# ZiyuanMa/MAPF_RL

Hardware: NVIDIA B200
Metric: env_agent_steps_per_sec_step_observe (higher is better)
Workload: dtype u8

## Files before the change

mapf_rl_b200/csrc/mapf_bfs_device.cuh:

```cuda
#pragma once
#include <type_traits>

#include "mapf_common.cuh"

namespace {

#ifdef MAPF_ENABLE_DIAG
__device__ unsigned long long g_bfs_cycles[8];
#endif

template <int RW, int RPL>
struct BfsState {
    uint32_t unv[RPL][RW];
    uint32_t fro[RPL][RW];
    uint32_t m1[RPL][RW];
    uint32_t m2[RPL][RW];
};

__device__ __forceinline__ uint32_t bfs_column_mask(int L, int w)
{
    const int lo = max(4 - 32 * w, 0), hi = min(L + 4 - 32 * w, 32);
    if (hi <= lo) return 0u;
    return (hi - lo == 32) ? 0xffffffffu : (((1u << (hi - lo)) - 1u) << lo);
}

template <int RW, int RPL>
struct BfsFree {
    uint32_t v[RPL][RW];
};

template <int RW, int RPL, int APW>
__device__ __forceinline__ void bfs_load_free(const EnvDims &d, const uint32_t *ob, BfsFree<RW, RPL> &F)
{
    constexpr int LW = 32 / APW;
    const int lane = (threadIdx.x & 31) % LW;
#pragma unroll
    for (int q = 0; q < RPL; ++q) {
        const int row = lane * RPL + q;
#pragma unroll
        for (int w = 0; w < RW; ++w)
            F.v[q][w] = (row < d.L) ? (~__ldcg(ob + (row + 4) * d.RWS + w) & bfs_column_mask(d.L, w)) : 0u;
    }
}

template <int RW, int RPL, int APW>
__device__ __forceinline__ void bfs_init(const EnvDims &d, const BfsFree<RW, RPL> &F, const int gx, const int gy, const bool alive,
                                         BfsState<RW, RPL> &S)
{
    constexpr int LW = 32 / APW;
    const int lane = (threadIdx.x & 31) % LW;
#pragma unroll
    for (int q = 0; q < RPL; ++q) {
        const int row = lane * RPL + q;
#pragma unroll
        for (int w = 0; w < RW; ++w) {
            const uint32_t fre = alive ? F.v[q][w] : 0u;
            const int p = gy + 4;
            S.fro[q][w] = (row == gx && (p >> 5) == w) ? ((1u << (p & 31)) & fre) : 0u;
            S.unv[q][w] = fre & ~S.fro[q][w];
            S.m1[q][w] = S.m2[q][w] = 0;
        }
    }
}

template <int RW, int RPL, int APW, bool WRAP>
__device__ __forceinline__ uint32_t bfs_wave(const BfsState<RW, RPL> &S, uint32_t (&nw)[RPL][RW])
{
    constexpr int LW = 32 / APW;
    const int lane = (threadIdx.x & 31) % LW;
    uint32_t any = 0;
#pragma unroll
    for (int w = 0; w < RW; ++w) {
        uint32_t above, below;
        if constexpr (WRAP) {
            above = __shfl_sync(MAPF_FULL_MASK, S.fro[RPL - 1][w], (lane + LW - 1) & (LW - 1), LW);
            below = __shfl_sync(MAPF_FULL_MASK, S.fro[0][w], (lane + 1) & (LW - 1), LW);
        } else {
            above = __shfl_up_sync(MAPF_FULL_MASK, S.fro[RPL - 1][w], 1, LW);
            below = __shfl_down_sync(MAPF_FULL_MASK, S.fro[0][w], 1, LW);
            if (lane == 0) above = 0;
            if (lane == LW - 1) below = 0;
        }
#pragma unroll
        for (int q = 0; q < RPL; ++q) {
            const uint32_t f = S.fro[q][w];
            const uint32_t fl = w > 0 ? __funnelshift_l(S.fro[q][w > 0 ? w - 1 : 0], f, 1) : f << 1;
            const uint32_t fr = w < RW - 1 ? __funnelshift_r(f, S.fro[q][w < RW - 1 ? w + 1 : w], 1) : f >> 1;
            const uint32_t up = q > 0 ? S.fro[q > 0 ? q - 1 : 0][w] : above;
            const uint32_t dn = q < RPL - 1 ? S.fro[q < RPL - 1 ? q + 1 : q][w] : below;
            const uint32_t x = (fl | fr | up | dn) & S.unv[q][w];
            nw[q][w] = x;
            any |= x;
        }
    }
    return any;
}

template <int RW, int RPL, int SEL>
__device__ __forceinline__ void bfs_apply(BfsState<RW, RPL> &S, const uint32_t (&nw)[RPL][RW])
{
#pragma unroll
    for (int q = 0; q < RPL; ++q)
#pragma unroll
        for (int w = 0; w < RW; ++w) {
            S.unv[q][w] -= nw[q][w];
            S.fro[q][w] = nw[q][w];
            if constexpr (SEL == 1) S.m1[q][w] += nw[q][w];
            if constexpr (SEL == 2) S.m2[q][w] += nw[q][w];
        }
}

template <int RW, int RPL, int APW, bool KEEP>
__device__ __forceinline__ void bfs_emit(const EnvDims &d, const uint32_t *ob, const BfsFree<RW, RPL> &F, const int e, const int a,
                                         const bool alive, const BfsState<RW, RPL> &S, uint32_t *__restrict__ navi)
{
    constexpr int LW = 32 / APW;
    const int lane = (threadIdx.x & 31) % LW;
    uint32_t pl[4][RPL][RW];
    uint32_t z[RPL][RW];
#pragma unroll
    for (int q = 0; q < RPL; ++q) {
        const int row = alive ? lane * RPL + q : d.L;
#pragma unroll
        for (int w = 0; w < RW; ++w) {
            uint32_t fre;
            if constexpr (KEEP) fre = alive ? F.v[q][w] : 0u;
            else fre = (row < d.L) ? (~__ldcg(ob + (row + 4) * d.RWS + w) & bfs_column_mask(d.L, w)) : 0u;
            z[q][w] = fre & ~S.unv[q][w] & ~S.m1[q][w] & ~S.m2[q][w];
        }
    }
    auto closer = [](uint32_t c1, uint32_t c2, uint32_t cz, uint32_t n1, uint32_t n2, uint32_t nz) -> uint32_t {
        return (c1 & nz) | (c2 & n1) | (cz & n2);
    };
#pragma unroll
    for (int w = 0; w < RW; ++w) {
        uint32_t a1 = __shfl_up_sync(MAPF_FULL_MASK, S.m1[RPL - 1][w], 1, LW), b1 = __shfl_down_sync(MAPF_FULL_MASK, S.m1[0][w], 1, LW);
        uint32_t a2 = __shfl_up_sync(MAPF_FULL_MASK, S.m2[RPL - 1][w], 1, LW), b2 = __shfl_down_sync(MAPF_FULL_MASK, S.m2[0][w], 1, LW);
        uint32_t az = __shfl_up_sync(MAPF_FULL_MASK, z[RPL - 1][w], 1, LW), bz = __shfl_down_sync(MAPF_FULL_MASK, z[0][w], 1, LW);
        if (lane == 0) a1 = a2 = az = 0;
        if (lane == LW - 1) b1 = b2 = bz = 0;
#pragma unroll
        for (int q = 0; q < RPL; ++q) {
            auto left = [&](const uint32_t(&m)[RPL][RW]) {
                return w > 0 ? __funnelshift_l(m[q][w > 0 ? w - 1 : 0], m[q][w], 1) : m[q][w] << 1;
            };
            auto right = [&](const uint32_t(&m)[RPL][RW]) {
                return w < RW - 1 ? __funnelshift_r(m[q][w], m[q][w < RW - 1 ? w + 1 : w], 1) : m[q][w] >> 1;
            };
            const uint32_t c1 = S.m1[q][w], c2 = S.m2[q][w], cz = z[q][w];
            const uint32_t u1 = q > 0 ? S.m1[q > 0 ? q - 1 : 0][w] : a1, u2 = q > 0 ? S.m2[q > 0 ? q - 1 : 0][w] : a2,
                           uz = q > 0 ? z[q > 0 ? q - 1 : 0][w] : az;
            const uint32_t d1 = q < RPL - 1 ? S.m1[q < RPL - 1 ? q + 1 : q][w] : b1, d2 = q < RPL - 1 ? S.m2[q < RPL - 1 ? q + 1 : q][w] : b2,
                           dz = q < RPL - 1 ? z[q < RPL - 1 ? q + 1 : q][w] : bz;
            pl[0][q][w] = closer(c1, c2, cz, u1, u2, uz);
            pl[1][q][w] = closer(c1, c2, cz, d1, d2, dz);
            pl[2][q][w] = closer(c1, c2, cz, left(S.m1), left(S.m2), left(z));
            pl[3][q][w] = closer(c1, c2, cz, right(S.m1), right(S.m2), right(z));
        }
    }
    uint2 *nv = reinterpret_cast<uint2 *>(navi + ((size_t)e * d.N + a) * d.navi_agent_stride);
#pragma unroll
    for (int q = 0; q < RPL; ++q) {
        const int row = lane * RPL + q;
        if (row >= d.L || !alive) continue;
        const int pr = row + 4, bx1 = pr >> 3, r1 = pr & 7;
#pragma unroll
        for (int by = 0; by < 4 * RW; ++by) {
            if (by >= d.NB) continue;
            constexpr int kLast = RW - 1;
            const int w = by >> 2;
            const int s = (by & 3) * 8;
            uint32_t f[4];
#pragma unroll
            for (int k = 0; k < 4; ++k)
                f[k] = __funnelshift_r(pl[k][q][w], w < kLast ? pl[k][q][w < kLast ? w + 1 : kLast] : 0u, s) & 0xffffu;
            const uint2 v = make_uint2(f[0] | (f[1] << 16), f[2] | (f[3] << 16));
            if (bx1 < d.NB) nv[((size_t)(bx1 * d.NB + by) << 4) + r1] = v;
            if (bx1 > 0) nv[((size_t)((bx1 - 1) * d.NB + by) << 4) + r1 + 8] = v;
        }
    }
}

template <int RW, int RPL, int APW, bool WRAP, bool DIST, bool KEEP>
__device__ __forceinline__ void bfs_navi_search(const EnvDims &d, const int e, const int a, const int i, const bool alive,
                                                const uint32_t *__restrict__ ob, const BfsFree<RW, RPL> &F, const int gx, const int gy,
                                                uint32_t *__restrict__ navi, int32_t *__restrict__ dist_out)
{
    constexpr int LW = 32 / APW;
    const int lane = (threadIdx.x & 31) % LW;
#ifdef MAPF_ENABLE_DIAG
    const long long tb0 = clock64();
    long long triples = 0;
#endif
    BfsState<RW, RPL> S;
    bfs_init<RW, RPL, APW>(d, F, gx, gy, alive, S);
#ifdef MAPF_ENABLE_DIAG
    const long long tb1 = clock64();
#endif

    int32_t *dist = nullptr;
    if constexpr (DIST) {
        dist = alive ? dist_out + ((size_t)i * d.N + a) * d.L * d.L : nullptr;
        for (int q = 0; q < RPL; ++q) {
            const int row = lane * RPL + q;
            if (dist && row < d.L)
                for (int y = 0; y < d.L; ++y) dist[row * d.L + y] = MAPF_DIST_UNREACHABLE;
        }
        __syncwarp();
#pragma unroll
        for (int q = 0; q < RPL; ++q)
#pragma unroll
            for (int w = 0; w < RW; ++w)
                if (dist && S.fro[q][w]) dist[gx * d.L + gy] = 0;
    }

    auto wave = [&](auto selc, const int t) -> uint32_t {
        constexpr int sel = decltype(selc)::value;
        uint32_t nw[RPL][RW];
        const uint32_t any = bfs_wave<RW, RPL, APW, WRAP>(S, nw);
        bfs_apply<RW, RPL, sel>(S, nw);
        if constexpr (DIST) {
#pragma unroll
            for (int q = 0; q < RPL; ++q)
#pragma unroll
                for (int w = 0; w < RW; ++w) {
                    uint32_t x = dist ? nw[q][w] : 0u;
                    while (x) {
                        int b = __ffs(x) - 1;
                        x &= x - 1;
                        dist[(lane * RPL + q) * d.L + (32 * w + b - 4)] = t;
                    }
                }
        }
        return any;
    };
    for (int t = 1;; t += 3) {
        wave(std::integral_constant<int, 1>{}, t);
        wave(std::integral_constant<int, 2>{}, t + 1);
        const uint32_t any = wave(std::integral_constant<int, 0>{}, t + 2);
#ifdef MAPF_ENABLE_DIAG
        ++triples;
#endif
        if (!__any_sync(MAPF_FULL_MASK, any != 0)) break;
    }
#ifdef MAPF_ENABLE_DIAG
    const long long tb2 = clock64();
#endif
    bfs_emit<RW, RPL, APW, KEEP>(d, ob, F, e, a, alive, S, navi);
#ifdef MAPF_ENABLE_DIAG
    if (e == 0 && (threadIdx.x & 31) == 0) {
        const long long tb3 = clock64();
        atomicAdd(&g_bfs_cycles[0], (unsigned long long)(tb1 - tb0));
        atomicAdd(&g_bfs_cycles[1], (unsigned long long)(tb2 - tb1));
        atomicAdd(&g_bfs_cycles[2], (unsigned long long)(tb3 - tb2));
        atomicAdd(&g_bfs_cycles[3], 1ull);
        atomicAdd(&g_bfs_cycles[4], (unsigned long long)triples);
    }
#endif
}

template <int RW, int RPL, int APW>
__device__ __forceinline__ void bfs_navi_warp(const EnvDims &d, const int e, const int a, const int i, const bool alive,
                                              const uint32_t *__restrict__ obst, const uint8_t *__restrict__ goal,
                                              uint32_t *__restrict__ navi, int32_t *__restrict__ dist_out)
{
    constexpr int LW = 32 / APW;
    const uint32_t *ob = obst + (size_t)e * d.obst_stride;
    const uchar2 gg = __ldcg(reinterpret_cast<const uchar2 *>(goal) + (size_t)e * d.N + a);
    BfsFree<RW, RPL> F;
    bfs_load_free<RW, RPL, APW>(d, ob, F);
    if (dist_out) bfs_navi_search<RW, RPL, APW, false, true, false>(d, e, a, i, alive, ob, F, gg.x, gg.y, navi, dist_out);
    else if (d.L < LW * RPL) bfs_navi_search<RW, RPL, APW, true, false, false>(d, e, a, i, alive, ob, F, gg.x, gg.y, navi, nullptr);
    else bfs_navi_search<RW, RPL, APW, false, false, false>(d, e, a, i, alive, ob, F, gg.x, gg.y, navi, nullptr);
}

template <int RW, int RPL, int APW>
__device__ __forceinline__ void bfs_navi_warp_pre(const EnvDims &d, const int e, const int a, const bool alive, const uint32_t *__restrict__ ob,
                                                  const BfsFree<RW, RPL> &F, const int gx, const int gy, uint32_t *__restrict__ navi)
{
    constexpr int LW = 32 / APW;
    if (d.L < LW * RPL) bfs_navi_search<RW, RPL, APW, true, false, true>(d, e, a, 0, alive, ob, F, gx, gy, navi, nullptr);
    else bfs_navi_search<RW, RPL, APW, false, false, true>(d, e, a, 0, alive, ob, F, gx, gy, navi, nullptr);
}

}
```

mapf_rl_b200/csrc/mapf_reset_device.cuh:

```cuda
#pragma once
#include "mapf_common.cuh"

namespace {


__device__ __forceinline__ uint4 philox4x32_10(uint4 c, uint2 k)
{
#pragma unroll
    for (int r = 0; r < 10; ++r) {
        const uint32_t hi0 = __umulhi(0xD2511F53u, c.x), lo0 = 0xD2511F53u * c.x;
        const uint32_t hi1 = __umulhi(0xCD9E8D57u, c.z), lo1 = 0xCD9E8D57u * c.z;
        c = make_uint4(hi1 ^ c.y ^ k.x, lo1, hi0 ^ c.w ^ k.y, lo0);
        k.x += 0x9E3779B9u;
        k.y += 0xBB67AE85u;
    }
    return c;
}

enum : uint32_t { PURPOSE_DENSITY = 0, PURPOSE_MAP = 1, PURPOSE_AGENT = 2, PURPOSE_LEVEL = 3 };

#ifdef MAPF_ENABLE_DIAG
__device__ unsigned long long g_reset_cycles[8];
#define MAPF_RESET_TICK(slot)                 \
    do {                                      \
        const long long _now = clock64();     \
        _acc[slot] += _now - _t0;             \
        _t0 = _now;                           \
    } while (0)
#else
#define MAPF_RESET_TICK(slot) do {} while (0)
#endif

template <int RW, int RPL>
struct Bits {
    uint32_t v[RPL][RW];
};

template <int RW, int RPL>
__device__ __forceinline__ void dilate(const Bits<RW, RPL> &f, Bits<RW, RPL> &out, int lane)
{
#pragma unroll
    for (int q = 0; q < RPL; ++q)
#pragma unroll
        for (int w = 0; w < RW; ++w) {
            const uint32_t x = f.v[q][w];
            uint32_t fl = x << 1, fr = x >> 1;
            if (w > 0) fl |= f.v[q][w > 0 ? w - 1 : 0] >> 31;
            if (w < RW - 1) fr |= f.v[q][w < RW - 1 ? w + 1 : w] << 31;
            uint32_t up = __shfl_up_sync(MAPF_FULL_MASK, x, 1);
            uint32_t dn = __shfl_down_sync(MAPF_FULL_MASK, x, 1);
            uint32_t wrap_up = 0, wrap_dn = 0;
            if (q > 0) wrap_up = __shfl_sync(MAPF_FULL_MASK, f.v[q > 0 ? q - 1 : 0][w], 31);
            if (q < RPL - 1) wrap_dn = __shfl_sync(MAPF_FULL_MASK, f.v[q < RPL - 1 ? q + 1 : q][w], 0);
            if (lane == 0) up = wrap_up;
            if (lane == 31) dn = wrap_dn;
            out.v[q][w] = fl | fr | up | dn;
        }
}

template <int RW, int RPL>
__device__ __forceinline__ int count_bits(const Bits<RW, RPL> &m)
{
    int c = 0;
#pragma unroll
    for (int q = 0; q < RPL; ++q)
#pragma unroll
        for (int w = 0; w < RW; ++w) c += __popc(m.v[q][w]);
    return c;
}

__device__ __forceinline__ int nth_set_bit(uint32_t m, int n)
{
    int pos = 0;
#pragma unroll
    for (int half = 16; half >= 1; half >>= 1) {
        const int c = __popc(m & ((1u << half) - 1u));
        if (n >= c) {
            n -= c;
            pos += half;
            m >>= half;
        }
    }
    return pos;
}

template <int RW, int RPL>
__device__ __forceinline__ int pick_bit(const Bits<RW, RPL> &m, uint32_t rnd, int lane, int &total_out)
{
    constexpr int kMax = 32 * RW * RPL;
    constexpr int kBits = kMax >= 512 ? 10 : (kMax >= 256 ? 9 : (kMax >= 128 ? 8 : (kMax >= 64 ? 7 : 6)));
    const int c = count_bits(m);
    const uint32_t lt = (1u << lane) - 1u;
    int excl = 0, total = 0;
#pragma unroll
    for (int k = 0; k < kBits; ++k) {
        const uint32_t b = __ballot_sync(MAPF_FULL_MASK, (c >> k) & 1);
        excl += __popc(b & lt) << k;
        total += __popc(b) << k;
    }
    total_out = total;
    if (total == 0) return -1;
    const int r = (int)__umulhi(rnd, (uint32_t)total);
    int local = r - excl;
    uint32_t code = 0;
    if (local >= 0 && local < c) {
        bool found = false;
#pragma unroll
        for (int q = 0; q < RPL; ++q)
#pragma unroll
            for (int w = 0; w < RW; ++w) {
                const int pc = __popc(m.v[q][w]);
                if (!found && local < pc) {
                    code = (uint32_t)((((lane + 32 * q) << 8) | (32 * w + nth_set_bit(m.v[q][w], local))) + 1);
                    found = true;
                }
                if (!found) local -= pc;
            }
    }
    return (int)__reduce_or_sync(MAPF_FULL_MASK, code) - 1;
}

template <int RW, int RPL>
__device__ __forceinline__ void clear_cell(Bits<RW, RPL> &m, int code, int lane)
{
    const int row = code >> 8, col = code & 0xff;
#pragma unroll
    for (int q = 0; q < RPL; ++q)
#pragma unroll
        for (int w = 0; w < RW; ++w)
            if (lane + 32 * q == row && (col >> 5) == w) m.v[q][w] &= ~(1u << (col & 31));
}

template <int RW, int RPL>
__device__ __forceinline__ bool test_cell(const Bits<RW, RPL> &m, int code, int lane)
{
    const int row = code >> 8, col = code & 0xff;
    bool hit = false;
#pragma unroll
    for (int q = 0; q < RPL; ++q)
#pragma unroll
        for (int w = 0; w < RW; ++w)
            if (lane + 32 * q == row && (col >> 5) == w) hit = (m.v[q][w] >> (col & 31)) & 1u;
    return __any_sync(MAPF_FULL_MASK, hit);
}

template <int RW, int RPL>
__device__ __forceinline__ void reset_env_warp(const EnvDims &d, const int e, const uint64_t seed, const uint64_t g,
                                               const float density, uint32_t *__restrict__ obst, uint8_t *__restrict__ pos,
                                               uint8_t *__restrict__ goal, int32_t *__restrict__ steps, int32_t *__restrict__ err,
                                               const int L, const int N)
{
    const int lane = threadIdx.x & 31;
    const int NS = d.N;
    const uint2 key = make_uint2((uint32_t)seed, (uint32_t)(seed >> 32));
    const uint32_t g_lo = (uint32_t)g, g_hi = (uint32_t)(g >> 32);

    float dens = density;
    if (density < 0.f) {
        const uint4 r = philox4x32_10(make_uint4(g_lo, g_hi, PURPOSE_DENSITY, 0u), key);
        const float u = (float)(r.x >> 8) * (1.0f / 16777216.0f);
        dens = u < 0.66f ? sqrtf(u * 0.5f * 0.33f) : 0.5f - sqrtf((1.0f - u) * 0.5f * 0.17f);
    }
    const uint32_t thresh = dens <= 0.f ? 0u : (dens >= 1.f ? 0xffffffffu : (uint32_t)((double)dens * 4294967296.0));

    Bits<RW, RPL> fre, elig, comp, big;
    int big_n = 0;
#ifdef MAPF_ENABLE_DIAG
    long long _t0 = clock64();
    long long _acc[8] = {0, 0, 0, 0, 0, 0, 0, 0};
#endif
    for (uint32_t attempt = 0;; ++attempt) {
        if (attempt >= 256) {
            if (lane == 0) atomicOr(err, MAPF_ERRBIT_RESET);
            break;
        }
#pragma unroll
        for (int q = 0; q < RPL; ++q) {
            const int row = lane + 32 * q;
#pragma unroll
            for (int w = 0; w < RW; ++w) fre.v[q][w] = 0;
            if (row < L) {
                for (int y4 = 0; y4 < L; y4 += 4) {
                    const uint4 r = philox4x32_10(make_uint4(g_lo, g_hi, PURPOSE_MAP | (attempt << 8), (uint32_t)(row * 64 + (y4 >> 2))), key);
                    uint32_t nib = (r.x >= thresh ? 1u : 0u) | (r.y >= thresh ? 2u : 0u) | (r.z >= thresh ? 4u : 0u) | (r.w >= thresh ? 8u : 0u);
                    if (y4 + 4 > L) nib &= (1u << (L - y4)) - 1u;
                    const int p = y4 + 4;
#pragma unroll
                    for (int w = 0; w < RW; ++w)
                        if ((p >> 5) == w) fre.v[q][w] |= nib << (p & 31);
                }
            }
        }
        MAPF_RESET_TICK(0);
        dilate(fre, elig, lane);
#pragma unroll
        for (int q = 0; q < RPL; ++q)
#pragma unroll
            for (int w = 0; w < RW; ++w) {
                elig.v[q][w] &= fre.v[q][w];
                comp.v[q][w] = 0;
                big.v[q][w] = 0;
            }
        big_n = 0;
        bool ok = true;
        MAPF_RESET_TICK(1);
        uint32_t draw_x[MAPF_MAX_AGENTS / 32], draw_y[MAPF_MAX_AGENTS / 32];
#pragma unroll
        for (int k = 0; k < MAPF_MAX_AGENTS / 32; ++k) {
            draw_x[k] = draw_y[k] = 0;
            if (k * 32 < N) {
                const uint4 r = philox4x32_10(make_uint4(g_lo, g_hi, PURPOSE_AGENT | (attempt << 8), (uint32_t)(k * 32 + lane)), key);
                draw_x[k] = r.x, draw_y[k] = r.y;
            }
        }
        for (int i = 0; i < N; ++i) {
            uint2 r = make_uint2(0u, 0u);
#pragma unroll
            for (int k = 0; k < MAPF_MAX_AGENTS / 32; ++k)
                if ((i >> 5) == k) r = make_uint2(__shfl_sync(MAPF_FULL_MASK, draw_x[k], i & 31), __shfl_sync(MAPF_FULL_MASK, draw_y[k], i & 31));
            MAPF_RESET_TICK(2);
            int total;
            const int s = pick_bit(elig, r.x, lane, total);
            MAPF_RESET_TICK(3);
            if (s < 0) {
                ok = false;
                break;
            }
            if (!test_cell(comp, s, lane) && big_n > 0 && test_cell(big, s, lane)) {
#pragma unroll
                for (int q = 0; q < RPL; ++q)
#pragma unroll
                    for (int w = 0; w < RW; ++w) comp.v[q][w] = big.v[q][w];
            } else if (!test_cell(comp, s, lane)) {
#pragma unroll
                for (int q = 0; q < RPL; ++q)
#pragma unroll
                    for (int w = 0; w < RW; ++w) comp.v[q][w] = 0;
                {
                    const int row = s >> 8, col = s & 0xff;
#pragma unroll
                    for (int q = 0; q < RPL; ++q)
#pragma unroll
                        for (int w = 0; w < RW; ++w)
                            if (lane + 32 * q == row && (col >> 5) == w) comp.v[q][w] = 1u << (col & 31);
                }
                for (;;) {
                    uint32_t grew = 0;
#pragma unroll
                    for (int rep = 0; rep < 4; ++rep) {
                        Bits<RW, RPL> nb;
                        dilate(comp, nb, lane);
                        grew = 0;
#pragma unroll
                        for (int q = 0; q < RPL; ++q)
#pragma unroll
                            for (int w = 0; w < RW; ++w) {
                                const uint32_t add = nb.v[q][w] & fre.v[q][w] & ~comp.v[q][w];
                                comp.v[q][w] |= add;
                                grew |= add;
                            }
                    }
                    if (!__any_sync(MAPF_FULL_MASK, grew != 0)) break;
                }
                const int n = __reduce_add_sync(MAPF_FULL_MASK, count_bits(comp));
                if (n > big_n) {
                    big_n = n;
#pragma unroll
                    for (int q = 0; q < RPL; ++q)
#pragma unroll
                        for (int w = 0; w < RW; ++w) big.v[q][w] = comp.v[q][w];
                }
            }
            MAPF_RESET_TICK(4);
            clear_cell(elig, s, lane);
            Bits<RW, RPL> cand;
#pragma unroll
            for (int q = 0; q < RPL; ++q)
#pragma unroll
                for (int w = 0; w < RW; ++w) cand.v[q][w] = elig.v[q][w] & comp.v[q][w];
            int cnt;
            const int t = pick_bit(cand, r.y, lane, cnt);
            clear_cell(elig, t, lane);
            if (cnt - 1 < 2) {
#pragma unroll
                for (int q = 0; q < RPL; ++q)
#pragma unroll
                    for (int w = 0; w < RW; ++w) elig.v[q][w] &= ~comp.v[q][w];
            }
            MAPF_RESET_TICK(5);
            if (lane == 0) {
                const size_t o = ((size_t)e * NS + i) * 2;
                pos[o] = (uint8_t)(s >> 8);
                pos[o + 1] = (uint8_t)((s & 0xff) - 4);
                goal[o] = (uint8_t)(t >> 8);
                goal[o + 1] = (uint8_t)((t & 0xff) - 4);
            }
            MAPF_RESET_TICK(6);
        }
        if (ok) break;
    }

    uint32_t *ob = obst + (size_t)e * d.obst_stride;
    for (int w = lane; w < d.obst_stride; w += 32) {
        const int prow = w / d.RWS;
        if (prow < 4 || prow >= L + 4 || w - prow * d.RWS >= RW) ob[w] = 0;
    }
#pragma unroll
    for (int q = 0; q < RPL; ++q) {
        const int row = lane + 32 * q;
        if (row < L) {
#pragma unroll
            for (int w = 0; w < RW; ++w) {
                const int lo = max(4 - 32 * w, 0), hi = min(L + 4 - 32 * w, 32);
                uint32_t cm = 0;
                if (hi > lo) cm = (hi - lo == 32) ? 0xffffffffu : (((1u << (hi - lo)) - 1u) << lo);
                ob[(row + 4) * d.RWS + w] = ~fre.v[q][w] & cm;
            }
        }
    }
    if (lane == 0) steps[e] = 0;
#ifdef MAPF_ENABLE_DIAG
    MAPF_RESET_TICK(7);
    if (e == 0 && lane == 0)
        for (int i = 0; i < 8; ++i) g_reset_cycles[i] = (unsigned long long)_acc[i];
#endif
}

template <int RW, int RPL>
__device__ __forceinline__ void reset_env_warp(const EnvDims &d, const int e, const uint64_t seed, const uint64_t g,
                                               const float density, uint32_t *__restrict__ obst, uint8_t *__restrict__ pos,
                                               uint8_t *__restrict__ goal, int32_t *__restrict__ steps, int32_t *__restrict__ err)
{
    reset_env_warp<RW, RPL>(d, e, seed, g, density, obst, pos, goal, steps, err, d.L, d.N);
}

}
```

mapf_rl_b200/csrc/mapf_rollout_kernels.cu:

```cuda
#include "mapf_rollout_device.cuh"

int mapf_launch_rollout_occ8(mapf_env *, const StepParams &, const void *, const void *, cudaStream_t);
int mapf_launch_rollout_occ10(mapf_env *, const StepParams &, const void *, const void *, cudaStream_t);
int mapf_launch_rollout_occ12(mapf_env *, const StepParams &, const void *, const void *, cudaStream_t);
int mapf_launch_rollout_occ16(mapf_env *, const StepParams &, const void *, const void *, cudaStream_t);

namespace {

RolloutTuning &rollout_tuning()
{
    static RolloutTuning t = [] {
        RolloutTuning r{0, 0, 0, 1000, 0};
        if (const char *s = std::getenv("MAPF_ROLLOUT_WARPS_PER_SM")) r.warps_per_sm = std::atoi(s);
        if (const char *s = std::getenv("MAPF_ROLLOUT_CHUNK")) r.chunk = std::atoi(s);
        if (const char *s = std::getenv("MAPF_ROLLOUT_STORE_MODE")) r.store_mode = std::atoi(s);
        if (const char *s = std::getenv("MAPF_ROLLOUT_STAGGER_NS")) r.stagger_ns = std::atoi(s);
        return r;
    }();
    return t;
}

}

void mapf_set_rollout_tuning(int warps_per_sm, int chunk, int store_mode, int stagger_ns)
{
    RolloutTuning &t = rollout_tuning();
    if (warps_per_sm >= 0) t.warps_per_sm = warps_per_sm;
    if (chunk >= 0) t.chunk = chunk;
    if (store_mode >= 0) t.store_mode = store_mode;
    if (stagger_ns >= 0) t.stagger_ns = stagger_ns;
}

bool mapf_rollout_supported(const mapf_env *env) { return env->d.K <= 2; }

int &rollout_pregen_ref()
{
    static int v = [] {
        const char *s = std::getenv("MAPF_ROLLOUT_PREGEN");
        return s ? std::atoi(s) : 1;
    }();
    return v;
}
void mapf_set_rollout_pregen(int on) { rollout_pregen_ref() = on; }
int &rollout_tasks_ref()
{
    static int v = [] {
        const char *s = std::getenv("MAPF_ROLLOUT_TASKS");
        return s ? std::atoi(s) : 0;
    }();
    return v;
}
void mapf_set_rollout_tasks(int on) { rollout_tasks_ref() = on; }
#ifdef MAPF_ENABLE_DIAG
static unsigned long long *g_trace = nullptr;
static int g_trace_cap = 0;
extern "C" int mapf_diag_rollout_trace(unsigned long long *d_buf, int capacity)
{
    g_trace = d_buf, g_trace_cap = capacity;
    return 0;
}
#endif
int mapf_launch_pregen(mapf_env *env, int min_count, cudaStream_t st);

int mapf_launch_rollout(mapf_env *env, int e0, int e1, int T, const uint8_t *d_actions, int action_slots, uint8_t *d_obs, int obs_slots,
                        const StepOut &out, int out_slots, cudaStream_t st)
{
    if (!mapf_rollout_supported(env)) return MAPF_EINVAL;
    StepParams p = mapf_make_step_params(env);
    p.env_begin = e0;
    p.env_end = e1;
    RolloutArgs r{};
    r.T = T, r.action_slots = action_slots, r.obs_slots = obs_slots, r.out_slots = out_slots;
    r.actions = d_actions, r.obs = d_obs, r.rewards = out.rewards, r.codes = out.codes, r.done = out.done, r.steps_out = out.steps;
    r.work = env->ro_work, r.progress = env->ro_progress;
    r.store_mode = rollout_tuning().store_mode;
    r.stagger_ns = rollout_tuning().stagger_ns;
    r.max_steps = env->ar_max_steps;
    r.seed = env->ar_seed, r.env_offset = env->ar_offset, r.stride = env->ar_stride, r.density = env->ar_density;
    r.episode = env->ro_episode;
#ifdef MAPF_ENABLE_DIAG
    r.trace = g_trace, r.trace_cap = g_trace_cap;
#endif
    static const int use_prio = [] { const char *v = std::getenv("MAPF_ROLLOUT_PRIO"); return v ? std::atoi(v) : 1; }();
    r.prio = nullptr, r.prio_flag = nullptr, r.pg_epi = nullptr, r.prio_last = 0;
    r.tq = nullptr;
    int reserve_ctas = 0;
    if (r.max_steps > 0) {
        if (rollout_tasks_ref()) r.tq = env->ro_tq, r.tq_cap = env->ro_tq_cap;
        const int mode = rollout_pregen_ref();
        const bool have_mem = env->navi_alt != nullptr;
        cudaStreamCaptureStatus cap = cudaStreamCaptureStatusNone;
        MAPF_CUDA(cudaStreamIsCapturing(st, &cap));
        const long long due = (long long)(e1 - e0) * (T < r.max_steps ? T : r.max_steps) / r.max_steps;
        bool before = false, beside = false;
        if (have_mem && mode != 0) {
            if (mode == 2) before = true;
            else if (mode == 3) beside = true;
            else if (due >= (long long)env->num_sms * 16) before = true;
            if (beside && cap != cudaStreamCaptureStatusNone) beside = false;
        }
        const bool prio = use_prio && T <= r.max_steps / 2;
        if (before || beside || prio) {
            rollout_prio_kernel<<<1, 1024, 0, st>>>(env->steps, e0, e1, T, r.max_steps, env->ro_prio, env->ro_prio_flag, env->pg_epi,
                                                    env->pg_cnt, env->ro_work);
            MAPF_CUDA(cudaGetLastError());
        }
        r.pregen_min = 0;
        if (before) {
            const int rc = mapf_launch_pregen(env, 0, st);
            if (rc != MAPF_OK) return rc;
        } else if (beside) {
            if (!env->pg_stream) {
                int lo = 0, hi = 0;
                MAPF_CUDA(cudaDeviceGetStreamPriorityRange(&lo, &hi));
                MAPF_CUDA(cudaStreamCreateWithPriority(&env->pg_stream, cudaStreamNonBlocking, hi));
                MAPF_CUDA(cudaEventCreateWithFlags(&env->pg_fork, cudaEventDisableTiming));
                MAPF_CUDA(cudaEventCreateWithFlags(&env->pg_join, cudaEventDisableTiming));
            }
            MAPF_CUDA(cudaEventRecord(env->pg_fork, st));
            MAPF_CUDA(cudaStreamWaitEvent(env->pg_stream, env->pg_fork, 0));
            const int rc = mapf_launch_pregen(env, 0, env->pg_stream);
            if (rc != MAPF_OK) return rc;
            MAPF_CUDA(cudaEventRecord(env->pg_join, env->pg_stream));
            r.prio_last = 1;
            static const int reserve = [] { const char *v = std::getenv("MAPF_ROLLOUT_RESERVE"); return v ? std::atoi(v) : 1; }();
            reserve_ctas = reserve;
        }
        if (before || beside) {
            r.pg_epi = env->pg_epi, r.pg_obst = env->pg_obst, r.pg_pos = env->pg_pos, r.pg_goal = env->pg_goal;
            r.navi_sel = env->navi_sel;
        }
        if (prio || beside) r.prio = env->ro_prio, r.prio_flag = env->ro_prio_flag;
    }
    const RolloutTuning &tn = rollout_tuning();
    const int want = tn.warps_per_sm > 0 ? tn.warps_per_sm : 16;
    RolloutTuning use = tn;
    use.warps_per_sm = want;
    use.reserve_ctas = reserve_ctas;
    int rc;
    if (want <= 16) rc = mapf_launch_rollout_occ8(env, p, &r, &use, st);
    else if (want <= 20) rc = mapf_launch_rollout_occ10(env, p, &r, &use, st);
    else if (want <= 24) rc = mapf_launch_rollout_occ12(env, p, &r, &use, st);
    else rc = mapf_launch_rollout_occ16(env, p, &r, &use, st);
    if (r.prio_last) MAPF_CUDA(cudaStreamWaitEvent(st, env->pg_join, 0));
    return rc;
}
```

Baseline: 10.12 billion.

## Cache pick-bit prefix counts across agents, pack navi bytes with byte_perm, disable stagger

The reset loop keeps warp-wide counts (per-lane count, exclusive prefix, total) for the eligible and candidate masks and updates them incrementally when a cell is cleared. This avoids redoing the multi-ballot recount on every pick. The BFS navi output packing replaces funnel-shift plus mask plus OR with __byte_perm for the byte-aligned cases. Separately, the stagger delay is set to zero when priority rollout is active. The incremental counts risk drifting out of sync with the masks, so an optional consistency check is included.

```diff
diff --git a/mapf_rl_b200/csrc/mapf_bfs_device.cuh b/mapf_rl_b200/csrc/mapf_bfs_device.cuh
--- a/mapf_rl_b200/csrc/mapf_bfs_device.cuh
+++ b/mapf_rl_b200/csrc/mapf_bfs_device.cuh
@@ -169,12 +169,13 @@
             if (by >= d.NB) continue;
             constexpr int kLast = RW - 1;
             const int w = by >> 2;
-            const int s = (by & 3) * 8;
-            uint32_t f[4];
-#pragma unroll
-            for (int k = 0; k < 4; ++k)
-                f[k] = __funnelshift_r(pl[k][q][w], w < kLast ? pl[k][q][w < kLast ? w + 1 : kLast] : 0u, s) & 0xffffu;
-            const uint2 v = make_uint2(f[0] | (f[1] << 16), f[2] | (f[3] << 16));
+            const int j = by & 3;
+            auto pack = [&](const uint32_t(&pa)[RPL][RW], const uint32_t(&pb)[RPL][RW]) -> uint32_t {
+                if (j < 3) return __byte_perm(pa[q][w], pb[q][w], (j | (j + 1) << 4 | (j + 4) << 8 | (j + 5) << 12));
+                const uint32_t na = w < kLast ? pa[q][w < kLast ? w + 1 : kLast] : 0u, nb = w < kLast ? pb[q][w < kLast ? w + 1 : kLast] : 0u;
+                return __byte_perm(__funnelshift_r(pa[q][w], na, 24), __funnelshift_r(pb[q][w], nb, 24), 0x5410);
+            };
+            const uint2 v = make_uint2(pack(pl[0], pl[1]), pack(pl[2], pl[3]));
             if (bx1 < d.NB) nv[((size_t)(bx1 * d.NB + by) << 4) + r1] = v;
             if (bx1 > 0) nv[((size_t)((bx1 - 1) * d.NB + by) << 4) + r1 + 8] = v;
         }
diff --git a/mapf_rl_b200/csrc/mapf_reset_device.cuh b/mapf_rl_b200/csrc/mapf_reset_device.cuh
--- a/mapf_rl_b200/csrc/mapf_reset_device.cuh
+++ b/mapf_rl_b200/csrc/mapf_reset_device.cuh
@@ -29,6 +29,10 @@
     } while (0)
 #else
 #define MAPF_RESET_TICK(slot) do {} while (0)
+#endif
+
+#ifdef MAPF_CHECK_PICK_COUNTS
+__device__ unsigned int g_pick_count_errors;
 #endif
 
 template <int RW, int RPL>
@@ -84,26 +88,46 @@
     return pos;
 }
 
-template <int RW, int RPL>
-__device__ __forceinline__ int pick_bit(const Bits<RW, RPL> &m, uint32_t rnd, int lane, int &total_out)
+struct PickCounts {
+    int c, excl, total;
+};
+
+template <int RW, int RPL>
+__device__ __forceinline__ PickCounts recount(const Bits<RW, RPL> &m, int lane)
 {
     constexpr int kMax = 32 * RW * RPL;
     constexpr int kBits = kMax >= 512 ? 10 : (kMax >= 256 ? 9 : (kMax >= 128 ? 8 : (kMax >= 64 ? 7 : 6)));
-    const int c = count_bits(m);
+    PickCounts p{count_bits(m), 0, 0};
     const uint32_t lt = (1u << lane) - 1u;
-    int excl = 0, total = 0;
 #pragma unroll
     for (int k = 0; k < kBits; ++k) {
-        const uint32_t b = __ballot_sync(MAPF_FULL_MASK, (c >> k) & 1);
-        excl += __popc(b & lt) << k;
-        total += __popc(b) << k;
-    }
-    total_out = total;
-    if (total == 0) return -1;
-    const int r = (int)__umulhi(rnd, (uint32_t)total);
-    int local = r - excl;
+        const uint32_t b = __ballot_sync(MAPF_FULL_MASK, (p.c >> k) & 1);
+        p.excl += __popc(b & lt) << k;
+        p.total += __popc(b) << k;
+    }
+    return p;
+}
+
+__device__ __forceinline__ void uncount(PickCounts &p, int code, int lane)
+{
+    const int owner = (code >> 8) & 31;
+    p.c -= lane == owner;
+    p.excl -= lane > owner;
+    p.total -= 1;
+}
+
+template <int RW, int RPL>
+__device__ __forceinline__ int pick_bit(const Bits<RW, RPL> &m, const PickCounts &p, uint32_t rnd, int lane)
+{
+#ifdef MAPF_CHECK_PICK_COUNTS
+    const PickCounts f = recount(m, lane);
+    if (__any_sync(MAPF_FULL_MASK, f.c != p.c || f.excl != p.excl || f.total != p.total) && lane == 0) atomicAdd(&g_pick_count_errors, 1u);
+#endif
+    if (p.total == 0) return -1;
+    const int r = (int)__umulhi(rnd, (uint32_t)p.total);
+    int local = r - p.excl;
     uint32_t code = 0;
-    if (local >= 0 && local < c) {
+    if (local >= 0 && local < p.c) {
         bool found = false;
 #pragma unroll
         for (int q = 0; q < RPL; ++q)
@@ -203,6 +227,8 @@
             }
         big_n = 0;
         bool ok = true;
+        PickCounts pe = recount(elig, lane), pc{0, 0, 0};
+        bool pc_valid = false;
         MAPF_RESET_TICK(1);
         uint32_t draw_x[MAPF_MAX_AGENTS / 32], draw_y[MAPF_MAX_AGENTS / 32];
 #pragma unroll
@@ -219,8 +245,7 @@
             for (int k = 0; k < MAPF_MAX_AGENTS / 32; ++k)
                 if ((i >> 5) == k) r = make_uint2(__shfl_sync(MAPF_FULL_MASK, draw_x[k], i & 31), __shfl_sync(MAPF_FULL_MASK, draw_y[k], i & 31));
             MAPF_RESET_TICK(2);
-            int total;
-            const int s = pick_bit(elig, r.x, lane, total);
+            const int s = pick_bit(elig, pe, r.x, lane);
             MAPF_RESET_TICK(3);
             if (s < 0) {
                 ok = false;
@@ -231,7 +256,9 @@
                 for (int q = 0; q < RPL; ++q)
 #pragma unroll
                     for (int w = 0; w < RW; ++w) comp.v[q][w] = big.v[q][w];
+                pc_valid = false;
             } else if (!test_cell(comp, s, lane)) {
+                pc_valid = false;
 #pragma unroll
                 for (int q = 0; q < RPL; ++q)
 #pragma unroll
@@ -273,19 +300,27 @@
             }
             MAPF_RESET_TICK(4);
             clear_cell(elig, s, lane);
+            uncount(pe, s, lane);
             Bits<RW, RPL> cand;
 #pragma unroll
             for (int q = 0; q < RPL; ++q)
 #pragma unroll
                 for (int w = 0; w < RW; ++w) cand.v[q][w] = elig.v[q][w] & comp.v[q][w];
-            int cnt;
-            const int t = pick_bit(cand, r.y, lane, cnt);
+            if (pc_valid) uncount(pc, s, lane);
+            else pc = recount(cand, lane);
+            pc_valid = true;
+            const int cnt = pc.total;
+            const int t = pick_bit(cand, pc, r.y, lane);
             clear_cell(elig, t, lane);
+            uncount(pe, t, lane);
+            uncount(pc, t, lane);
             if (cnt - 1 < 2) {
 #pragma unroll
                 for (int q = 0; q < RPL; ++q)
 #pragma unroll
                     for (int w = 0; w < RW; ++w) elig.v[q][w] &= ~comp.v[q][w];
+                pe = recount(elig, lane);
+                pc_valid = false;
             }
             MAPF_RESET_TICK(5);
             if (lane == 0) {
diff --git a/mapf_rl_b200/csrc/mapf_rollout_kernels.cu b/mapf_rl_b200/csrc/mapf_rollout_kernels.cu
--- a/mapf_rl_b200/csrc/mapf_rollout_kernels.cu
+++ b/mapf_rl_b200/csrc/mapf_rollout_kernels.cu
@@ -131,6 +131,7 @@
             r.navi_sel = env->navi_sel;
         }
         if (prio || beside) r.prio = env->ro_prio, r.prio_flag = env->ro_prio_flag;
+        if (prio) r.stagger_ns = 0;
     }
     const RolloutTuning &tn = rollout_tuning();
     const int want = tn.warps_per_sm > 0 ? tn.warps_per_sm : 16;
```

Result: faster. 10.43 billion (median of 6 runs) (+3.0%).
